# avi2924/Speech-Intent-Recognizer

Hardware: AMD Instinct MI355X
Metric: utterances/sec (16 kHz, 3 s clips), inference: HIP STFT+mel+CNN/BiGRU forward + argmax (higher is better)
Workload: dtype f32

## Files before the change

speech-intent-recognizer_amd/csrc/conv_fwd.h:

```cpp
#pragma once
#include "conv_wino2_f16x3_kernel.h"

template <int CIN, int COUT, int OUT_MODE>
static inline int conv_fwd(sir_handle* h, hipStream_t st, bool wino, const Wino2Geo& geo, int nb, const float* x, const unsigned short* w_wino,
                           const unsigned short* w_fallback, const float* scale, const float* shift, float* out, float2* stats,
                           const int* ctab = nullptr, int ncol_max = 0) {
    static_assert((CIN == 32 && COUT == 64) || (CIN == 64 && COUT == 128), "conv2 or conv3");
    const int H = geo.H, W = geo.W;
    if (wino) {
        SIR_TRY(sir_lds_opt_in(h, (const void*)conv3x3_wino2_f16x3_kernel<CIN, COUT, OUT_MODE, 0, 3>, W2_LDS_BYTES));
        SIR_HIP_TRY((launch_conv_wino2<CIN, COUT, OUT_MODE>(st, geo, x, w_wino, scale, shift, out, stats, h->zero_page, h->num_cus, ctab, ncol_max)));
    } else if constexpr (CIN == 32) {
        hipLaunchKernelGGL((conv3x3_wino_bf16x6_kernel<CIN, COUT, OUT_MODE == 2 ? 2 : 0>), dim3(((W + 1) / 2 + 1) / 2, 1, nb), dim3(256), WINO_LDS_BYTES, st,
                           x, w_wino, scale, shift, out, H, W, H / 2, W / 2, OUT_MODE == 2 ? stats : (float2*)nullptr);
    } else {
        hipLaunchKernelGGL((conv3x3_bf16x6_ns_kernel<CIN, COUT, 2, 2, OUT_MODE, 0, 2, 1, 1>), dim3((W + 7) / 8, 1, nb), dim3(256), conv_ns_lds_bytes(2, 2, 2), st,
                           x, w_fallback, scale, shift, out, H, W, H / 2, W / 2, stats);
    }
    return SIR_OK;
}
```

speech-intent-recognizer_amd/csrc/conv_wino2_f16x3_kernel.h:

```cpp
#pragma once
#include "conv_wino_bf16x6_kernel.h"
#include "wino2_geo.h"

constexpr int W2_RS = 11;
constexpr int W2_NPOS = 18 * W2_RS;
constexpr int W2_RAW_PIECES = (W2_NPOS * 4 + 63) / 64;
constexpr int W2_RAW_BYTES = W2_RAW_PIECES * 1024;
constexpr int W2_PLB = 16 * 1024;
constexpr int W2_NRAW = 3;
constexpr int W2_V_BYTES = 2 * W2_PLB;
constexpr int W2_XCH_BYTES = 3 * W2_PLB;
constexpr int W2_LDS_BYTES = 2 * W2_V_BYTES + W2_NRAW * W2_RAW_BYTES + W2_XCH_BYTES;
constexpr int W2_THREADS = 768;
constexpr int W2_PPW = (W2_RAW_PIECES + 3) / 4;

__device__ __forceinline__ int w2_div(int n, const W2Div& d) {
    const unsigned un = (unsigned)n;
    if (d.pow2) return (int)(un >> d.sh);
    const unsigned t = __umulhi(d.m, un);
    return (int)((t + ((un - t) >> 1)) >> d.sh);
}

__device__ __forceinline__ void split_w_f16x3(float u, unsigned short& p0, unsigned short& p1, unsigned int* status) {
    constexpr float LIM = 31.984375f;
    if (status && !(fabsf(u) <= LIM)) __hip_atomic_fetch_or(status, 8u, __ATOMIC_RELAXED, __HIP_MEMORY_SCOPE_AGENT);
    u = __builtin_fminf(__builtin_fmaxf(u, -LIM), LIM);
    const _Float16 hi = (_Float16)u;
    const _Float16 lo = (_Float16)((u - (float)hi) * H3_LO_SCALE);
    p0 = __builtin_bit_cast(unsigned short, hi);
    p1 = __builtin_bit_cast(unsigned short, lo);
}
__device__ __forceinline__ void prep_conv_w_wino_f16x3_elem(const float* __restrict__ w, unsigned short* __restrict__ wpb, int cin, int cout, int idx,
                                                            unsigned int* status) {
    const int total = cin * 16 * cout;
    if (idx >= total) return;
    const int e = idx & 15, co = (idx >> 4) % cout, g = (idx >> 4) / cout;
    const int ci = (g / 16) * 16 + e, f = g % 16, i = f >> 2, j = f & 3;
    const float* gk = w + ((size_t)co * cin + ci) * 9;
    const float Gm[4][3] = {{1.f, 0.f, 0.f}, {.5f, .5f, .5f}, {.5f, -.5f, .5f}, {0.f, 0.f, 1.f}};
    float u = 0.0f;
#pragma unroll
    for (int k = 0; k < 3; ++k) {
        float t = 0.0f;
#pragma unroll
        for (int l = 0; l < 3; ++l) t = fmaf(gk[k * 3 + l], Gm[j][l], t);
        u = fmaf(Gm[i][k], t, u);
    }
    if (j == 3) u = -u;
    split_w_f16x3(u, wpb[idx], wpb[(size_t)total + idx], status);
}
static __global__ void prep_conv_w_wino_f16x3_kernel(const float* __restrict__ w, unsigned short* __restrict__ wpb, int cin, int cout,
                                                     unsigned int* status) {
    prep_conv_w_wino_f16x3_elem(w, wpb, cin, cout, blockIdx.x * blockDim.x + threadIdx.x, status);
}
__device__ __forceinline__ void prep_conv_wT_wino_f16x3_elem(const float* __restrict__ w, unsigned short* __restrict__ wpb, int cin_f, int cout_f,
                                                             int idx, unsigned int* status) {
    const int total = cout_f * 16 * cin_f;
    if (idx >= total) return;
    const int e = idx & 15, cop = (idx >> 4) % cin_f, g = (idx >> 4) / cin_f;
    const int co_f = (g / 16) * 16 + e, f = g % 16, i = f >> 2, j = f & 3;
    const float* gk = w + ((size_t)co_f * cin_f + cop) * 9;
    const float Gm[4][3] = {{1.f, 0.f, 0.f}, {.5f, .5f, .5f}, {.5f, -.5f, .5f}, {0.f, 0.f, 1.f}};
    float u = 0.0f;
#pragma unroll
    for (int k = 0; k < 3; ++k) {
        float t = 0.0f;
#pragma unroll
        for (int l = 0; l < 3; ++l) t = fmaf(gk[8 - (k * 3 + l)], Gm[j][l], t);
        u = fmaf(Gm[i][k], t, u);
    }
    if (j == 3) u = -u;
    split_w_f16x3(u, wpb[idx], wpb[(size_t)total + idx], status);
}
static __global__ void prep_conv_wT_wino_f16x3_kernel(const float* __restrict__ w, unsigned short* __restrict__ wpb, int cin_f, int cout_f,
                                                       unsigned int* status) {
    prep_conv_wT_wino_f16x3_elem(w, wpb, cin_f, cout_f, blockIdx.x * blockDim.x + threadIdx.x, status);
}

typedef float w2_f32x4 __attribute__((ext_vector_type(4)));
typedef unsigned w2_u32x2 __attribute__((ext_vector_type(2)));
__device__ __forceinline__ void w2_barrier() { asm volatile("s_waitcnt lgkmcnt(0)\n\ts_barrier" ::: "memory"); }
__device__ __forceinline__ void w2_read_row(unsigned base, w2_f32x4& r0, w2_f32x4& r1, w2_f32x4& r2, w2_f32x4& r3) {
    asm volatile("ds_read_b128 %0, %4\n\tds_read_b128 %1, %4 offset:64\n\tds_read_b128 %2, %4 offset:128\n\tds_read_b128 %3, %4 offset:192"
                 : "=&v"(r0), "=&v"(r1), "=&v"(r2), "=&v"(r3) : "v"(base) : "memory");
}
template <int OFF>
__device__ __forceinline__ void w2_write64(unsigned base, uint2 v) {
    const w2_u32x2 d = {v.x, v.y};
    asm volatile("ds_write_b64 %0, %1 offset:%2" :: "v"(base), "v"(d), "n"(OFF) : "memory");
}

__device__ long long w2_dbg_stamps[2][32];
__device__ long long w2_dbg_fine[8][8];
template <int CIN, int COUT, int OUT_MODE, int DBG = 0, int PRIO = 3>
__global__ __launch_bounds__(W2_THREADS, 3) void conv3x3_wino2_f16x3_kernel(
    const float* __restrict__ x, const unsigned short* __restrict__ wpb, const float* __restrict__ scale,
    const float* __restrict__ shift, float* __restrict__ out, Wino2Geo geo, float2* __restrict__ stats, const float* __restrict__ zeros) {
    constexpr int NCH = CIN / 16, G = NCH * 16, NCHO = COUT >= 64 ? COUT / 64 : 1;
    static_assert(CIN % 16 == 0 && (COUT % 64 == 0 || COUT == 32), "16-channel chunks; 64-channel tasks (32: the n = 1 consumer waves only keep the barriers)");
    static_assert(NCH >= 2, "a task's exchange pieces are read behind its closing barrier; the next task's are written >= one barrier later");
    extern __shared__ __attribute__((aligned(1024))) unsigned char w2s[];
    constexpr int VB = W2_V_BYTES;
    unsigned char* const vbuf = w2s;
    unsigned char* const rawbuf = w2s + 2 * VB;
    unsigned char* const xchbuf = rawbuf + W2_NRAW * W2_RAW_BYTES;

    const int tid = threadIdx.x, lane = tid & 63, wv = __builtin_amdgcn_readfirstlane(tid >> 6);
    const bool producer = wv < 4;
    const int H = geo.H, W = geo.W, TW = geo.TW, NG = geo.NG, RBN = geo.RBN;
    const int* const ctab = OUT_MODE <= 1 ? geo.ctab : nullptr;
    const int NS = ctab ? RBN * ctab[0] : geo.NS;
    const int ntask_s = (NS - (int)blockIdx.x + (int)gridDim.x - 1) / (int)gridDim.x;
    const int ntask = ntask_s * NCHO;
    if (ntask <= 0) return;
    const int nsteps = ntask * NCH;

    auto task_geo = [&](int lt, int& g0, int& ty0, int& ch, int& s) {
        s = (int)blockIdx.x + (lt / NCHO) * (int)gridDim.x;
        ch = lt % NCHO;
        const int cb = w2_div(s, geo.dRBN), rb = s - cb * RBN;
        g0 = ctab ? ctab[1 + cb] : 4 * cb; ty0 = 8 * rb;
    };
    constexpr bool IDLE_DMA = COUT < 64;
    constexpr int D_STRIDE = 4, D_PPW = (W2_RAW_PIECES + D_STRIDE - 1) / D_STRIDE;
    const int d_stride = D_STRIDE;
    const int d_rank = producer ? wv : ((wv - 4) >> 1);
    int pre_lr[D_PPW], pre_lc[D_PPW], pre_part[D_PPW];
#pragma unroll
    for (int ii = 0; ii < D_PPW; ++ii) {
        const int slot = 64 * (d_rank + d_stride * ii) + lane, pos = slot >> 2, sp = slot & 3;
        const int lr = pos / W2_RS;
        const int lc = pos - lr * W2_RS - ((lr >> 1) & 1);
        const bool hole = lr > 17 || lc < 0 || lc > 9;
        pre_lr[ii] = hole ? (1 << 20) : lr;
        pre_lc[ii] = lc;
        pre_part[ii] = (sp ^ (((lr >> 2) & 1) << 1)) * 4;
    }
    auto raw_offsets = [&](int g0, int ty0, unsigned (&off)[D_PPW]) {
        const int plo = ctab ? 2 * TW * w2_div(g0, geo.dTW) : 0, phi = ctab ? plo + W : 2 * NG;
#pragma unroll
        for (int ii = 0; ii < D_PPW; ++ii) {
            const int gy = 2 * ty0 - 1 + pre_lr[ii];
            const int P = 2 * g0 - 1 + pre_lc[ii];
            const int Pc = min(max(P, 0), 2 * NG - 1);
            const int bb = w2_div(Pc, geo.d2TW), px = Pc - bb * 2 * TW;
            const bool ok = gy >= 0 && gy < H && P >= plo && P < phi && px < W;
            off[ii] = ok ? (unsigned)(((bb * H + gy) * W + px) * CIN + pre_part[ii]) : ~0u;
        }
    };
        auto raw_issue = [&](const unsigned (&off)[D_PPW], int c, int slot_buf) {
#pragma unroll
        for (int ii = 0; ii < D_PPW; ++ii) {
            const int k = d_rank + d_stride * ii;
            if (k < W2_RAW_PIECES) {
                const float* src = off[ii] == ~0u ? zeros : x + off[ii];
                __builtin_amdgcn_global_load_lds((sir_gptr_t)(src + c * 16), (sir_lptr_t)(rawbuf + slot_buf * W2_RAW_BYTES + k * 1024), 16, 0, 0);
            }
        }
    };
    int ig0, ity0, ich, is_;
    unsigned roff[D_PPW];
    int roff_task = -1;
    auto issue_chunk = [&](int q) {
        if (q >= nsteps) return;
        const int lt = q / NCH, c = q - lt * NCH;
        if (lt != roff_task) { task_geo(lt, ig0, ity0, ich, is_); raw_offsets(ig0, ity0, roff); roff_task = lt; }
        raw_issue(roff, c, q % W2_NRAW);
    };
    int nst = 0;
    auto stamp = [&]() {
        if (DBG && blockIdx.x == 0 && lane == 0 && (wv == 0 || wv == 4) && nst < 32) w2_dbg_stamps[producer ? 0 : 1][nst] = __builtin_amdgcn_s_memtime();
        ++nst;
    };

    if (producer) {
        if (PRIO) __builtin_amdgcn_s_setprio(PRIO);
        __builtin_amdgcn_s_setreg((1 ) | (23 << 6) | (0 << 11), 1);
        const int wg = wv;
        const int tR = wg >> 1, tH = wg & 1, tm = lane >> 1, tP1 = lane & 1;
        const int tty = tm & 7, ttx = tm >> 3, tpart = 2 * tH + tP1;
        unsigned ra_rel[3];
#pragma unroll
        for (int rr = 0; rr < 3; ++rr) {
            const int lr = 2 * tty + tR + rr;
            ra_rel[rr] = (unsigned)((lr * W2_RS + 2 * ttx + ((lr >> 1) & 1)) * 64 + ((tpart ^ (((lr >> 2) & 1) << 1)) * 16));
        }
        const unsigned raw_a = (unsigned)(uintptr_t)rawbuf, v_a = (unsigned)(uintptr_t)vbuf + (8 * tR) * 1024 + tH * 512 + tm * 16 + tP1 * 8;
        if (!IDLE_DMA) {
            issue_chunk(0);
            issue_chunk(1);
            asm volatile("s_waitcnt vmcnt(0)" ::: "memory");
        }
        w2_barrier();
        bool edge = false, z0 = false, z3 = false;
        auto fine = [&](int s_, int k_) {
            if (DBG && blockIdx.x == 0 && lane == 0 && wv == 0 && s_ >= 8 && s_ < 16) w2_dbg_fine[s_ - 8][k_] = __builtin_amdgcn_s_memtime();
        };
#pragma unroll 1
        for (int s = 0; s <= nsteps; ++s) {
            stamp();
            fine(s, 0);
            if (s < nsteps) {
                if (!IDLE_DMA && !(DBG & 2)) issue_chunk(s + 2);
                fine(s, 1);
                if (s % NCH == 0) {
                    int cg0, cty0, cch, cs;
                    task_geo(s / NCH, cg0, cty0, cch, cs);
                    const int t0 = cg0 - w2_div(cg0, geo.dTW) * TW;
                    edge = !ctab && (t0 == 0 || t0 + 3 >= TW - 1);
                    const int txx = (t0 + ttx) - w2_div(t0 + ttx, geo.dTW) * TW;
                    z0 = txx == 0; z3 = txx == TW - 1;
                }
                const unsigned rb = raw_a + (s % W2_NRAW) * W2_RAW_BYTES, vd = v_a + (s & 1) * VB;
                if (!(DBG & 4)) {
                w2_f32x4 q[3][4];
#pragma unroll
                for (int rr = 0; rr < 3; ++rr) w2_read_row(rb + ra_rel[rr], q[rr][0], q[rr][1], q[rr][2], q[rr][3]);
                asm volatile("s_waitcnt lgkmcnt(0)" ::: "memory");
                fine(s, 2);
                if (edge) {
                    asm volatile("" ::: "memory");
                    const w2_f32x4 zero4 = {0.0f, 0.0f, 0.0f, 0.0f};
#pragma unroll
                    for (int rr = 0; rr < 3; ++rr) { q[rr][0] = z0 ? zero4 : q[rr][0]; q[rr][3] = z3 ? zero4 : q[rr][3]; }
                }
                auto rows = [&](auto trc) {
                    constexpr int TR = decltype(trc)::value;
#pragma unroll
                    for (int il = 0; il < 2; ++il) {
                        w2_f32x4 R[4];
#pragma unroll
                        for (int j = 0; j < 4; ++j) {
                            if (TR == 0) R[j] = il == 0 ? q[0][j] - q[2][j] : q[1][j] + q[2][j];
                            else         R[j] = il == 0 ? q[1][j] - q[0][j] : q[0][j] - q[2][j];
                        }
                        const w2_f32x4 V[4] = {R[0] - R[2], R[1] + R[2], R[2] - R[1], R[1] - R[3]};
#pragma unroll
                        for (int j = 0; j < 4; ++j) {
                            const unsigned d = vd + (4 * il + j) * 1024;
                            uint2 sh, sl;
                            split2h_pair_ovfl(V[j].x, V[j].y, sh.x, sl.x);
                            split2h_pair_ovfl(V[j].z, V[j].w, sh.y, sl.y);
                            w2_write64<0>(d, sh);
                            w2_write64<W2_PLB>(d, sl);
                        }
                    }
                };
                if (tR == 0) rows(std::integral_constant<int, 0>{});
                else rows(std::integral_constant<int, 1>{});
                if (DBG) asm volatile("s_waitcnt lgkmcnt(0)" ::: "memory");
                fine(s, 3);
                }
                if (!IDLE_DMA) {
                    if (s + 2 < nsteps) asm volatile("s_waitcnt vmcnt(%0)" :: "n"(W2_RAW_PIECES / 4) : "memory");
                    else asm volatile("s_waitcnt vmcnt(0)" ::: "memory");
                }
            }
            stamp();
            fine(s, 4);
            w2_barrier();
            fine(s, 5);
        }
        return;
    }

    const int cw = wv - 4, mn = cw & 1, mi = cw >> 1, m = lane & 31, h = lane >> 5;
    if (COUT < 64 && mn == 1) {
        if (IDLE_DMA) {
            if (!(DBG & 2)) { issue_chunk(0); issue_chunk(1); }
            asm volatile("s_waitcnt vmcnt(0)" ::: "memory");
            w2_barrier();
#pragma unroll 1
            for (int s = 0; s <= nsteps; ++s) {
                if (s < nsteps) {
                    if (!(DBG & 2)) issue_chunk(s + 2);
                    if (s + 2 < nsteps) asm volatile("s_waitcnt vmcnt(%0)" :: "n"(W2_RAW_PIECES / 4) : "memory");
                    else asm volatile("s_waitcnt vmcnt(0)" ::: "memory");
                }
                w2_barrier();
            }
            return;
        }
        w2_barrier();
        w2_barrier();
        for (int lt = 0; lt < ntask; ++lt)
            for (int c = 0; c < NCH; ++c) w2_barrier();
        return;
    }
    const unsigned wlane = (unsigned)((m * 2 + h) * 16);
    const unsigned char* const wbase = reinterpret_cast<const unsigned char*>(wpb) + (size_t)mn * 1024;
    constexpr int NPW = 2;
    uint4 wq[4][NPW];
    auto load_w = [&](int gidx, int chh, uint4 (&q)[NPW]) {
#pragma unroll
        for (int p = 0; p < NPW; ++p)
            q[p] = *reinterpret_cast<const uint4*>(wbase + ((size_t)(p * G + gidx) * (COUT * 2) + (size_t)chh * 128) * 16 + wlane);
    };
    int g0, ty0, ch, s_idx;
    task_geo(0, g0, ty0, ch, s_idx);
#pragma unroll
    for (int j = 0; j < 4; ++j) load_w(4 * mi + j, ch, wq[j]);
    f32x16 acc[4];
#pragma unroll
    for (int j = 0; j < 4; ++j)
#pragma unroll
        for (int r = 0; r < 16; ++r) acc[j][r] = 0.0f;
    w2_barrier();
    float run_s[NCHO], run_q[NCHO];
#pragma unroll
    for (int k = 0; k < NCHO; ++k) { run_s[k] = 0.0f; run_q[k] = 0.0f; }

    stamp();
    stamp();
    w2_barrier();
#pragma unroll 1
    for (int lt = 0; lt < ntask; ++lt) {
        int g0n = g0, ty0n = ty0, chn = ch, sn = s_idx;
        if (lt + 1 < ntask) task_geo(lt + 1, g0n, ty0n, chn, sn);
#pragma unroll 1
        for (int c = 0; c < NCH; ++c) {
            stamp();
            const int sc = lt * NCH + c;
            const bool task_end = c == NCH - 1;
            const unsigned char* abase = vbuf + (sc & 1) * VB + h * 512 + m * 16 + (4 * mi) * 1024;
            const int gnxt = (task_end ? 0 : c + 1) * 16 + 4 * mi;
#pragma unroll
            for (int jp = 0; jp < 2; ++jp) {
                constexpr int NPA = 2;
                bf16x8 a[2][NPA], bq[2][3];
#pragma unroll
                for (int jj = 0; jj < 2; ++jj) {
#pragma unroll
                    for (int p = 0; p < NPA; ++p)
                        a[jj][p] = __builtin_bit_cast(bf16x8, *reinterpret_cast<const uint4*>(abase + p * W2_PLB + (2 * jp + jj) * 1024));
                    const f16x8 uh = __builtin_bit_cast(f16x8, wq[2 * jp + jj][0]);
                    bq[jj][0] = __builtin_bit_cast(bf16x8, uh);
                    bq[jj][1] = __builtin_bit_cast(bf16x8, uh * (_Float16)2048.0f);
                    bq[jj][2] = __builtin_bit_cast(bf16x8, wq[2 * jp + jj][1]);
                }
                if (DBG & 8) {
#pragma unroll
                    for (int jj = 0; jj < 2; ++jj)
                        acc[2 * jp + jj][0] += __builtin_bit_cast(float4, a[jj][0]).x + __builtin_bit_cast(float4, a[jj][1]).y + __builtin_bit_cast(float4, a[jj][NPA - 1]).z +
                                               __builtin_bit_cast(float4, bq[jj][0]).x + __builtin_bit_cast(float4, bq[jj][1]).y + __builtin_bit_cast(float4, bq[jj][2]).z;
                } else {
                    constexpr int HA[3] = {1, 0, 0}, HB[3] = {0, 2, 1};
#pragma unroll
                    for (int t3 = 0; t3 < 3; ++t3)
#pragma unroll
                        for (int jj = 0; jj < 2; ++jj)
                            acc[2 * jp + jj] = __builtin_amdgcn_mfma_f32_32x32x16_f16(__builtin_bit_cast(f16x8, a[jj][HA[t3]]),
                                                                                      __builtin_bit_cast(f16x8, bq[jj][HB[t3]]), acc[2 * jp + jj], 0, 0, 0);
                }
#pragma unroll
                for (int jj = 0; jj < 2; ++jj) if (!(DBG & 64)) load_w(gnxt + 2 * jp + jj, task_end ? chn : ch, wq[2 * jp + jj]);
                __builtin_amdgcn_sched_barrier(0);
            }
            stamp();
            if (!task_end) w2_barrier();
        }
        if (DBG & 16) { w2_barrier(); if (acc[0][0] == 1234.5f && acc[1][1] + acc[2][2] + acc[3][3] == 4.0f) out[0] = 1.0f; }
        else {
            {
                float4* const xch = reinterpret_cast<float4*>(xchbuf);
                float own[2][4];
#pragma unroll
                for (int b = 0; b < 2; ++b) {
                    const f32x16 Wc = b == 0 ? acc[0] + acc[1] + acc[2] : acc[1] - acc[2] + acc[3];
#pragma unroll
                    for (int k = 0; k < 4; ++k) {
                        if (k == mi) {
#pragma unroll
                            for (int e = 0; e < 4; ++e) own[b][e] = Wc[4 * k + e];
                        } else {
                            float4* dst = xch + (size_t)((mn * 4 + mi) * 3 + ((k - mi - 1) & 3)) * 128 + lane;
                            dst[b * 64] = make_float4(Wc[4 * k], Wc[4 * k + 1], Wc[4 * k + 2], Wc[4 * k + 3]);
                        }
                    }
                }
                w2_barrier();
                float Y[2][2][4];
#pragma unroll
                for (int i = 0; i < 4; ++i) {
                    const int kk = (mi - i - 1) & 3;
                    const float4* src = xch + (size_t)((mn * 4 + i) * 3 + (kk < 3 ? kk : 0)) * 128 + lane;
#pragma unroll
                    for (int b = 0; b < 2; ++b) {
                        const float4 v = src[b * 64];
                        const float w[4] = {i == mi ? own[b][0] : v.x, i == mi ? own[b][1] : v.y, i == mi ? own[b][2] : v.z, i == mi ? own[b][3] : v.w};
#pragma unroll
                        for (int e = 0; e < 4; ++e) {
                            if (i == 0) Y[0][b][e] = w[e];
                            else if (i <= 2) Y[0][b][e] += w[e];
                            if (i == 1) Y[1][b][e] = w[e];
                            else if (i >= 2) Y[1][b][e] -= w[e];
                        }
                    }
                }
                const int co = ch * 64 + mn * 32 + m;
                float ssum = 0.0f, ssq = 0.0f;
                float sc_ = 1.0f, sh_ = 0.0f;
                constexpr float DESC = H3_LO_INV;
                if (OUT_MODE <= 1) { sc_ = scale[co] * DESC; sh_ = shift[co]; }
                {
                    const int gc = g0 + mi;
                    const int img = w2_div(gc, geo.dTW), tx = gc - img * TW;
                    const bool tvalid = gc < (ctab ? (w2_div(g0, geo.dTW) + 1) * TW : NG);
                    if (OUT_MODE <= 1) {
                        float pooled[4];
#pragma unroll
                        for (int e = 0; e < 4; ++e) {
                            float v = 0.0f;
#pragma unroll
                            for (int a = 0; a < 2; ++a)
#pragma unroll
                                for (int b = 0; b < 2; ++b) v = fmaxf(v, fmaf(Y[a][b][e], sc_, sh_));
                            pooled[e] = v;
                        }
                        if (tvalid && tx < geo.Wp) {
                            if (OUT_MODE == 0) {
#pragma unroll
                                for (int e = 0; e < 4; ++e)
                                    out[(((size_t)img * geo.Hp + ty0 + 4 * h + e) * geo.Wp + tx) * COUT + co] = pooled[e];
                            } else {
                                const size_t oidx = ((size_t)img * geo.Wp + tx) * (COUT * geo.Hp) + (size_t)co * geo.Hp + ty0 + 4 * h;
                                const float4 v4 = make_float4(pooled[0], pooled[1], pooled[2], pooled[3]);
                                *reinterpret_cast<float4*>(out + oidx) = v4;
                                if (stats) {
                                    unsigned short* planes = reinterpret_cast<unsigned short*>(stats);
                                    const size_t plane = (size_t)geo.B * geo.Wp * (COUT * geo.Hp);
                                    uint2 hh, ll;
                                    split2h_quad(v4, hh, ll);
                                    *reinterpret_cast<uint2*>(planes + oidx) = hh;
                                    *reinterpret_cast<uint2*>(planes + plane + oidx) = ll;
                                }
                            }
                        }
                    } else {
#pragma unroll
                        for (int e = 0; e < 4; ++e)
#pragma unroll
                            for (int a = 0; a < 2; ++a)
#pragma unroll
                                for (int b = 0; b < 2; ++b) {
                                    const int gy = 2 * (ty0 + 4 * h + e) + a, gx = 2 * tx + b;
                                    if (tvalid && gx < W) {
                                        const float v = Y[a][b][e] * DESC;
                                        out[(((size_t)img * H + gy) * W + gx) * COUT + co] = v;
                                        ssum += v;
                                        ssq = fmaf(v, v, ssq);
                                    }
                                }
                    }
                }
                if (OUT_MODE == 2) {
#pragma unroll
                    for (int k = 0; k < NCHO; ++k)
                        if (k == ch) { run_s[k] += ssum; run_q[k] += ssq; }
                }
            }
        }
        g0 = g0n; ty0 = ty0n; ch = chn; s_idx = sn;
#pragma unroll
        for (int j = 0; j < 4; ++j)
#pragma unroll
            for (int r = 0; r < 16; ++r) acc[j][r] = 0.0f;
    }
    if (OUT_MODE == 2 && stats) {
#pragma unroll
        for (int k = 0; k < NCHO; ++k) {
            float a = run_s[k], q = run_q[k];
            a += __shfl_xor(a, 32);
            q += __shfl_xor(q, 32);
            if (h == 0) stats[((size_t)blockIdx.x * 4 + mi) * COUT + k * 64 + mn * 32 + m] = make_float2(a, q);
        }
    }
}

template <int CIN, int COUT, int OUT_MODE, int DBG = 0, int PRIO = 3>
static inline hipError_t launch_conv_wino2(hipStream_t st, Wino2Geo g, const float* x, const unsigned short* wpb, const float* scale,
                                           const float* shift, float* out, float2* stats, const float* zeros, int max_wg = 256,
                                           const int* ctab = nullptr, int ncol_max = 0) {
    if (ctab) {
        if (OUT_MODE > 1 || ncol_max < 1) return hipErrorInvalidValue;
        g.ctab = ctab;
        g.NS = g.RBN * ncol_max;
    }
    const int nwg = g.NS < max_wg ? g.NS : max_wg;
    hipLaunchKernelGGL((conv3x3_wino2_f16x3_kernel<CIN, COUT, OUT_MODE, DBG, PRIO>), dim3(nwg), dim3(W2_THREADS), W2_LDS_BYTES, st, x, wpb, scale, shift, out, g, stats, zeros);
    return hipGetLastError();
}
```

speech-intent-recognizer_amd/csrc/model_infer.hip:

```cpp
#include "f16x3_kernels.h"
#include "conv_fwd.h"
#include "gru_frag_prep.h"

namespace {

enum WsBuf {
    WS_A1 = 0,
    WS_A2,
    WS_X0,
    WS_GI,
    WS_Y0,
    WS_Y1,
    WS_CTX,
    WS_PAD,
    WS_XZ,
    WS_BN,
    WS_WHT,
    WS_XS,
    WS_WS,
    WS_WCB,
    WS_GXB,
    WS_GFL,
    WS_COUNT
};

struct Dims : SirDims {
    int tw2, tw3, k2max, k3max;
};

bool make_dims(int batch, int t_frames, Dims* d) {
    if (!sir_make_dims(batch, t_frames, d)) return false;
    d->tw2 = (d->wp1 + 1) / 2; d->tw3 = (d->wp2 + 1) / 2; d->k2max = (d->tw2 + 3) / 4; d->k3max = (d->tw3 + 3) / 4;
    return true;
}

struct PadTabs { size_t e0, d1, d3, tab2, tab3, rows, count; };
PadTabs pad_tabs(const Dims& d) {
    PadTabs t;
    const size_t n = (size_t)d.B + 1;
    t.e0 = 0; t.d1 = d.B; t.d3 = t.d1 + n; t.tab2 = t.d3 + n; t.tab3 = t.tab2 + 1 + n * d.k2max; t.rows = t.tab3 + 1 + n * d.k3max;
    t.count = t.rows + 1 + n * d.S;
    return t;
}

void ws_sizes(const Dims& d, size_t* bytes) {
    const size_t B = d.B + 1;
    bytes[WS_A1] = B * 32 * d.wp1 * 32 * 4;
    bytes[WS_A2] = B * 16 * d.wp2 * 64 * 4;
    bytes[WS_X0] = B * d.S * 1024 * 4;
    bytes[WS_GI] = B * d.S * 1536 * 4;
    bytes[WS_Y0] = (size_t)d.B * d.S * 512 * 4;
    bytes[WS_Y1] = (size_t)d.B * d.S * 512 * 4;
    bytes[WS_CTX] = (size_t)d.B * 512 * 4;
    bytes[WS_PAD] = pad_tabs(d).count * 4;
    bytes[WS_XZ] = (size_t)64 * d.T * 4;
    bytes[WS_BN] = (size_t)2 * 224 * 4;
    bytes[WS_WHT] = 4 * GRU_FRAG_BYTES;
    bytes[WS_XS] = B * d.S * 1024 * 2 * 2;
    bytes[WS_WS] = ((size_t)2 * 2 * 768 * 1024 + (size_t)2 * 2 * 768 * 512) * 2;
    bytes[WS_WCB] = ((size_t)3 * 32 * 16 * 64 + (size_t)3 * 64 * 16 * 128 + (size_t)3 * 64 * 9 * 128) * 2;
    bytes[WS_GXB] = 0;
    bytes[WS_GFL] = 0;
}

size_t ws_layout(const Dims& d, size_t* off) {
    size_t bytes[WS_COUNT], pos = 0;
    ws_sizes(d, bytes);
    for (int i = 0; i < WS_COUNT; ++i) {
        off[i] = pos;
        pos += sir_align_up(bytes[i], 256);
    }
    return pos;
}

static __global__ __launch_bounds__(256) void pad_extent_kernel(const float* __restrict__ x, int T, int* __restrict__ e0) {
    const unsigned* xb = reinterpret_cast<const unsigned*>(x) + (size_t)blockIdx.x * 64 * T;
    int last = -1;
    for (int c = threadIdx.x; c < T; c += 256) {
        unsigned acc = 0;
#pragma unroll 32
        for (int r = 0; r < 64; ++r) acc |= xb[(size_t)r * T + c];
        if (acc) last = c;
    }
#pragma unroll
    for (int o = 32; o > 0; o >>= 1) last = max(last, __shfl_xor(last, o));
    __shared__ int wl[4];
    if ((threadIdx.x & 63) == 0) wl[threadIdx.x >> 6] = last;
    __syncthreads();
    if (threadIdx.x == 0) e0[blockIdx.x] = max(max(wl[0], wl[1]), max(wl[2], wl[3])) + 1;
}

static __global__ __launch_bounds__(1024) void pad_tables_kernel(const int* __restrict__ e0, Dims d, int* __restrict__ d1o, int* __restrict__ d3o,
                                                                 int* __restrict__ tab2, int* __restrict__ tab3, int* __restrict__ prow,
                                                                 float* __restrict__ xz) {
    const int tid = threadIdx.x;
    for (int i = tid; i < 64 * d.T; i += 1024) xz[i] = 0.0f;
    const int nu = d.B + 1, per = (nu + 1023) / 1024, u0 = min(nu, tid * per), u1 = min(nu, u0 + per);
    auto need = [&](int u, int& c1, int& c3, int& k2, int& k3) {
        if (u == d.B) { c1 = d.wp1; c3 = d.S; k2 = d.k2max; k3 = d.k3max; return; }
        c3 = min(d.S, (e0[u] + 14) / 8);
        const int c2 = min(d.wp2, 2 * c3 + 1);
        c1 = min(d.wp1, 2 * c2 + 1);
        k2 = (c2 + 3) / 4; k3 = (c3 + 3) / 4;
    };
    int s2 = 0, s3 = 0, sr = 0, c1, c3, k2, k3;
    for (int u = u0; u < u1; ++u) { need(u, c1, c3, k2, k3); s2 += k2; s3 += k3; sr += c3; }
    __shared__ int p2[1024], p3[1024], pr[1024];
    p2[tid] = s2; p3[tid] = s3; pr[tid] = sr;
    __syncthreads();
    for (int o = 1; o < 1024; o <<= 1) {
        const int a2 = tid >= o ? p2[tid - o] : 0, a3 = tid >= o ? p3[tid - o] : 0, ar = tid >= o ? pr[tid - o] : 0;
        __syncthreads();
        p2[tid] += a2; p3[tid] += a3; pr[tid] += ar;
        __syncthreads();
    }
    int o2 = p2[tid] - s2, o3 = p3[tid] - s3, orw = pr[tid] - sr;
    for (int u = u0; u < u1; ++u) {
        need(u, c1, c3, k2, k3);
        d1o[u] = c1; d3o[u] = c3;
        for (int k = 0; k < k2; ++k) tab2[1 + o2 + k] = u * d.tw2 + 4 * k;
        for (int k = 0; k < k3; ++k) tab3[1 + o3 + k] = u * d.tw3 + 4 * k;
        for (int s = 0; s < c3; ++s) prow[1 + orw + s] = u * d.S + s;
        o2 += k2; o3 += k3; orw += c3;
    }
    if (tid == 1023) { tab2[0] = p2[1023]; tab3[0] = p3[1023]; prow[0] = pr[1023]; }
}

}

extern "C" size_t sir_model_workspace_bytes(const sir_handle* h, int batch, int t_frames, int train) {
    (void)h;
    if (train) return sir_train_workspace_bytes_impl(batch, t_frames);
    Dims d;
    if (!make_dims(batch, t_frames, &d)) return 0;
    size_t off[WS_COUNT];
    return ws_layout(d, off);
}

extern "C" int sir_model_workspace_offsets(const sir_handle* h, int batch, int t_frames, int train, size_t* offsets,
                                           int n) {
    (void)h; (void)train;
    Dims d;
    if (!make_dims(batch, t_frames, &d) || !offsets) { sir_set_error("sir_model_workspace_offsets: bad shape"); return SIR_EINVAL; }
    size_t off[WS_COUNT];
    ws_layout(d, off);
    for (int i = 0; i < n && i < WS_COUNT; ++i) offsets[i] = off[i];
    return WS_COUNT;
}

extern "C" int sir_model_infer(sir_handle* h, const sir_model_weights* w, const float* feats, int batch, int t_frames,
                               float* logits, int64_t* argmax, void* workspace, size_t workspace_bytes, void* stream_) {
    if (!h || !w || !feats || !logits || !workspace) { sir_set_error("sir_model_infer: NULL argument"); return SIR_EINVAL; }
    Dims d;
    if (!make_dims(batch, t_frames, &d)) {
        sir_set_error("sir_model_infer: unsupported shape batch=%d t_frames=%d (need t_frames >= 8)", batch, t_frames);
        return SIR_EINVAL;
    }
    if (h->cfg.n_mels != 64) { sir_set_error("sir_model_infer: the model is wired for 64 mels (models.py:23)"); return SIR_EUNSUPPORTED; }
    if (w->num_classes < 1 || w->num_classes > 64) { sir_set_error("sir_model_infer: num_classes=%d", w->num_classes); return SIR_EINVAL; }
    size_t off[WS_COUNT];
    const size_t need = ws_layout(d, off);
    if (workspace_bytes < need) { sir_set_error("sir_model_infer: workspace %zu < %zu", workspace_bytes, need); return SIR_ENOMEM; }
    if (((uintptr_t)workspace & 255) != 0) { sir_set_error("sir_model_infer: workspace must be 256-byte aligned"); return SIR_EINVAL; }
    hipStream_t st = (hipStream_t)stream_;
    char* ws = (char*)workspace;
    float* a1 = (float*)(ws + off[WS_A1]);
    float* a2 = (float*)(ws + off[WS_A2]);
    float* x0 = (float*)(ws + off[WS_X0]);
    float* gi = (float*)(ws + off[WS_GI]);
    float* y0 = (float*)(ws + off[WS_Y0]);
    float* y1 = (float*)(ws + off[WS_Y1]);
    float* ctx = (float*)(ws + off[WS_CTX]);
    float* bns = (float*)(ws + off[WS_BN]);
    float* bnt = bns + 224;
    float* wht = (float*)(ws + off[WS_WHT]);
    unsigned short* xs = (unsigned short*)(ws + off[WS_XS]);
    unsigned short* wsl0 = (unsigned short*)(ws + off[WS_WS]);
    unsigned short* wsl1 = wsl0 + (size_t)2 * 2 * 768 * 1024;
    unsigned short* wcb2 = (unsigned short*)(ws + off[WS_WCB]);
    unsigned short* wcb3 = wcb2 + (size_t)3 * 32 * 16 * 64;
    unsigned short* wcb3d = wcb3 + (size_t)3 * 64 * 16 * 128;
    const int B = d.B, S = d.S;
    const PadTabs pt = pad_tabs(d);
    int* const ptab = (int*)(ws + off[WS_PAD]);
    float* const xz = (float*)(ws + off[WS_XZ]);

    const SirConvPlan cp = sir_conv_plan(&d, true);
    const bool w2 = cp.fwd_wino;
    const int BT = w2 ? B + 1 : B;

    const long long prep_key = ((long long)B << 32) | (unsigned)d.T;
    sir_handle::PrepEntry* pe = nullptr;
    for (auto& e : h->prep)
        if (e.ws == workspace) pe = &e;
    const bool reuse_prep = pe && h->weights_version != 0 && pe->version == h->weights_version && pe->key == prep_key;
    if (!reuse_prep) {
        SirProfScope prof(h, SIR_K_PREP, st);
        const int bn_c[3] = {32, 64, 128}, bn_o[3] = {0, 32, 96};
        for (int i = 0; i < 3; ++i)
            hipLaunchKernelGGL(prep_bn_kernel, dim3(1), dim3(128), 0, st, w->bn_w[i], w->bn_b[i], w->bn_mean[i], w->bn_var[i],
                               bns + bn_o[i], bnt + bn_o[i], bn_c[i]);
        for (int i = 0; i < 4; ++i) sir_prep_whh_quad(st, w->gru_w_hh[i], (unsigned char*)wht + (size_t)i * GRU_FRAG_BYTES);
        if (w2) hipLaunchKernelGGL(prep_conv_w_wino_f16x3_kernel, dim3((32 * 16 * 64 + 255) / 256), dim3(256), 0, st, w->conv_w[1], wcb2, 32, 64, h->status);
        else hipLaunchKernelGGL(prep_conv_w_wino_bf16x3_kernel, dim3((32 * 16 * 64 + 255) / 256), dim3(256), 0, st, w->conv_w[1], wcb2, 32, 64);
        if (w2) hipLaunchKernelGGL(prep_conv_w_wino_f16x3_kernel, dim3((64 * 16 * 128 + 255) / 256), dim3(256), 0, st, w->conv_w[2], wcb3, 64, 128, h->status);
        else hipLaunchKernelGGL(prep_conv_w_wino_bf16x3_kernel, dim3((64 * 16 * 128 + 255) / 256), dim3(256), 0, st, w->conv_w[2], wcb3, 64, 128);
        hipLaunchKernelGGL(prep_conv_w_bf16x3_kernel, dim3((64 * 9 * 128 + 255) / 256), dim3(256), 0, st, w->conv_w[2], wcb3d, 64, 128);
        for (int dir = 0; dir < 2; ++dir) {
            hipLaunchKernelGGL(split2h_kernel, dim3(384), dim3(256), 0, st, w->gru_w_ih[dir], 1024, wsl0 + (size_t)dir * 2 * 768 * 1024, (size_t)768, 1024);
            hipLaunchKernelGGL(split2h_kernel, dim3(192), dim3(256), 0, st, w->gru_w_ih[2 + dir], 512, wsl1 + (size_t)dir * 2 * 768 * 512, (size_t)768, 512);
        }
        if (!pe) { pe = &h->prep[h->prep_next]; h->prep_next = (h->prep_next + 1) % 4; }
        pe->ws = workspace; pe->version = h->weights_version; pe->key = prep_key;
    }
    SIR_KCHECK();

    {
        SirProfScope prof(h, SIR_K_CONV1, st);
        if (w2) {
            hipLaunchKernelGGL(pad_extent_kernel, dim3(B), dim3(256), 0, st, feats, d.T, ptab + pt.e0);
            hipLaunchKernelGGL(pad_tables_kernel, dim3(1), dim3(1024), 0, st, (const int*)(ptab + pt.e0), d, ptab + pt.d1, ptab + pt.d3,
                               ptab + pt.tab2, ptab + pt.tab3, ptab + pt.rows, xz);
        }
        hipLaunchKernelGGL(conv1_mfma_bn_relu_pool_kernel, dim3((d.wp1 + C1_PCOLS - 1) / C1_PCOLS, 1, BT), dim3(256), 0, st, feats,
                           w->conv_w[0], bns, bnt, a1, 64, d.T, 32, d.wp1, (const float*)xz, B, w2 ? (const int*)(ptab + pt.d1) : (const int*)nullptr);
    }
    {
        SirProfScope prof(h, SIR_K_CONV2, st);
        SIR_TRY((conv_fwd<32, 64, 0>(h, st, w2, cp.geo2, BT, a1, wcb2, nullptr, bns + 32, bnt + 32, a2, nullptr, ptab + pt.tab2, (B + 1) * d.k2max)));
    }
    {
        SirProfScope prof(h, SIR_K_CONV3, st);
        SIR_TRY((conv_fwd<64, 128, 1>(h, st, w2, cp.geo3, BT, a2, wcb3, wcb3d, bns + 96, bnt + 96, x0, (float2*)xs, ptab + pt.tab3, (B + 1) * d.k3max)));
    }
    SIR_KCHECK();

    const int M = B * S;
    {
        SirProfScope prof(h, SIR_K_GEMM_IH0, st);
        if (w2)
            SIR_TRY(launch_gemm_nt_f16x3_gather(h, st, (const unsigned short*)xs, (const unsigned short*)wsl0,
                                                    (const unsigned short*)(wsl0 + (size_t)2 * 768 * 1024), w->gru_b_ih[0], w->gru_b_ih[1], gi, 1536,
                                                    (const int*)(ptab + pt.rows), BT * S, 768, 1024));
        else
            SIR_TRY(launch_gemm_nt_f16x3(h, st, (const unsigned short*)xs, (const unsigned short*)wsl0,
                                             (const unsigned short*)(wsl0 + (size_t)2 * 768 * 1024), w->gru_b_ih[0], w->gru_b_ih[1], gi, 1536, M, 768, 1024));
    }
    {
        SirProfScope prof(h, SIR_K_GRU0, st);
        SIR_TRY(sir_launch_gru_quad(h, st, false, gi, w->gru_w_hh[0], w->gru_w_hh[1], w->gru_b_hh[0], w->gru_b_hh[1], y0, B, S, nullptr,
                                    xs, wht, (unsigned char*)wht + GRU_FRAG_BYTES, w2 ? (const int*)(ptab + pt.d3) : (const int*)nullptr));
    }
    {
        SirProfScope prof(h, SIR_K_GEMM_IH1, st);
        SIR_TRY(launch_gemm_nt_f16x3(h, st, (const unsigned short*)xs, (const unsigned short*)wsl1,
                                         (const unsigned short*)(wsl1 + (size_t)2 * 768 * 512), w->gru_b_ih[2], w->gru_b_ih[3], gi, 1536, M, 768, 512));
    }
    {
        SirProfScope prof(h, SIR_K_GRU1, st);
        SIR_TRY(sir_launch_gru_quad(h, st, false, gi, w->gru_w_hh[2], w->gru_w_hh[3], w->gru_b_hh[2], w->gru_b_hh[3], y1, B, S, nullptr,
                                    nullptr, (unsigned char*)wht + 2 * GRU_FRAG_BYTES, (unsigned char*)wht + 3 * GRU_FRAG_BYTES));
    }
    SIR_KCHECK();

    {
        SirProfScope prof(h, SIR_K_ATTN, st);
        hipLaunchKernelGGL(attention_pool_kernel, dim3(B), dim3(256), 0, st, y1, w->attn_w, w->attn_b, ctx, S, w->fc_w, w->fc_b,
                           w->num_classes, logits, (long long*)argmax);
    }
    SIR_KCHECK();
    return SIR_OK;
}
```

speech-intent-recognizer_amd/csrc/wino2_geo.h:

```cpp
#pragma once
#include <stddef.h>

struct W2Div { unsigned m; int sh; int pow2; unsigned d; };
static inline W2Div w2_div_make(unsigned d) {
    W2Div r{0u, 0, 0, d};
    if ((d & (d - 1)) == 0) { r.pow2 = 1; while ((1u << r.sh) < d) ++r.sh; return r; }
    int l = 0;
    while ((1ull << l) < d) ++l;
    r.m = (unsigned)((((1ull << l) - d) << 32) / d + 1);
    r.sh = l - 1;
    return r;
}

struct Wino2Geo {
    int H, W;
    int TW;
    int NG;
    int RBN;
    int NS;
    int Hp, Wp;
    int B;
    W2Div dTW, d2TW, dRBN;
    const int* ctab;
};
static inline bool wino2_geo(int B, int H, int W, int cmax, Wino2Geo* g) {
    g->B = B; g->H = H; g->W = W; g->TW = (W + 1) / 2; g->NG = B * g->TW; g->RBN = H / 16; g->ctab = nullptr;
    g->NS = g->RBN * ((g->NG + 3) / 4); g->Hp = H / 2; g->Wp = W / 2;
    g->dTW = w2_div_make((unsigned)g->TW); g->d2TW = w2_div_make(2u * (unsigned)g->TW); g->dRBN = w2_div_make((unsigned)(g->RBN > 0 ? g->RBN : 1));
    return H % 16 == 0 && W >= 1 && B >= 1 && (size_t)B * H * W * cmax < ((size_t)1 << 31) && (size_t)g->NG * 2 < ((size_t)1 << 30);
}
static inline size_t wino2_stat_blocks(int B, int H, int W, int max_wg) {
    const size_t ns = (size_t)(H / 16) * (((size_t)B * ((W + 1) / 2) + 3) / 4);
    return (ns < (size_t)max_wg ? ns : (size_t)max_wg) * 4;
}
```

Baseline: 739,000.

## Dynamically claim Winograd conv tasks via a global atomic counter

Replaces the static strided task assignment in the persistent Winograd conv kernel with dynamic work stealing. After two statically assigned tasks, each workgroup claims further tasks through a global atomic counter. One lane issues the claim two chunks ahead and publishes it to a small LDS ring, so the fetch overlaps with the DMA pipeline. The counters are zeroed in the pad-tables kernel. This targets load imbalance from the padded/compacted column tables, at the cost of atomic traffic, an extra vmcnt slot and LDS reads per task. It also adds a trace-analysis script.

```diff
diff --git a/devtools/trace_pipeline.py b/devtools/trace_pipeline.py
--- /dev/null
+++ b/devtools/trace_pipeline.py
@@ -0,0 +1,128 @@
+import csv
+import statistics
+import sys
+from collections import defaultdict
+
+SEGMENT_GAP_NS = 2_000_000
+
+
+def short(name):
+    n = name.replace("(anonymous namespace)::", "")
+    if n.startswith("void "):
+        n = n[5:]
+    n = n.split("(")[0]
+    return n[:64]
+
+
+def load(path):
+    rows = list(csv.DictReader(open(path)))
+    key = "Stream_Id" if rows and "Stream_Id" in rows[0] and len({r["Stream_Id"] for r in rows}) > 1 else "Queue_Id"
+    ev = [(int(r["Start_Timestamp"]), int(r["End_Timestamp"]), short(r["Kernel_Name"]), r[key]) for r in rows]
+    ev.sort()
+    return ev, key
+
+
+def overlaps(ev):
+    out = []
+    by_start = ev
+    for i, (s, e, n, q) in enumerate(by_start):
+        ov = gru = False
+        j = i - 1
+        while j >= 0 and by_start[j][0] > s - 5_000_000:
+            s2, e2, n2, q2 = by_start[j]
+            if q2 != q and e2 > s:
+                ov = True
+                gru = gru or n2.startswith("gru_quad_kernel")
+            j -= 1
+        j = i + 1
+        while not ov and j < len(by_start) and by_start[j][0] < e:
+            ov = by_start[j][3] != q
+            j += 1
+        out.append((ov, gru))
+    return out
+
+
+def sweep(ev, t0, t1):
+    pts = []
+    for s, e, n, _ in ev:
+        if e <= t0 or s >= t1:
+            continue
+        g = n.startswith("gru_quad_kernel")
+        pts.append((max(s, t0), 1, g))
+        pts.append((min(e, t1), -1, g))
+    pts.sort(key=lambda p: (p[0], p[1]))
+    idle = only = 0
+    act = gact = 0
+    prev = t0
+    for t, d, g in pts:
+        if act == 0:
+            idle += t - prev
+        elif act == gact:
+            only += t - prev
+        act += d
+        gact += d if g else 0
+        prev = t
+    idle += t1 - prev
+    return idle, only
+
+
+def main(path):
+    ev, key = load(path)
+    ovl = overlaps(ev)
+    open_b = defaultdict(list)
+    batches = []
+    for i, (s, e, n, q) in enumerate(ev):
+        open_b[q].append(i)
+        if n.startswith("attention_pool_kernel"):
+            idx = open_b.pop(q)
+            batches.append((ev[idx[0]][0], e, q, idx))
+    batches.sort(key=lambda b: b[1])
+    piped = [b for b in batches if any(ovl[i][0] for i in b[3])]
+    if not piped:
+        sys.exit("no batch overlaps a kernel of another stream: not a pipelined trace")
+    segs, cur = [], [piped[0]]
+    for b in piped[1:]:
+        if b[1] - cur[-1][1] > SEGMENT_GAP_NS:
+            segs.append(cur)
+            cur = []
+        cur.append(b)
+    segs.append(cur)
+    segs = [s for s in segs if len(s) >= 4]
+    nb = sum(len(s) - 1 for s in segs)
+    wall = sum(s[-1][1] - s[0][1] for s in segs)
+    idle = only = 0
+    for s in segs:
+        a, b = sweep(ev, s[0][1], s[-1][1])
+        idle += a
+        only += b
+    print(f"streams keyed by {key}; {len(batches)} batches, {len(piped)} pipelined in {len(segs)} segments")
+    print(f"pipelined, per batch: wall {wall / nb / 1e3:.1f} us, nothing running {idle / nb / 1e3:.1f} us, "
+          f"only gru_quad_kernel running {only / nb / 1e3:.1f} us")
+    per = defaultdict(lambda: [0, 0])
+    conv = defaultdict(lambda: {"ovl": [], "alone": [], "beside_gru": 0, "n": 0})
+    seg_batches = {id(b) for s in segs for b in s[1:]}
+    for b in batches:
+        for i in b[3]:
+            s, e, n, q = ev[i]
+            if id(b) in seg_batches:
+                per[n][0] += e - s
+                per[n][1] += 1
+            if n.startswith("conv3x3_wino2_f16x3_kernel"):
+                c = conv[n]
+                (c["ovl"] if ovl[i][0] else c["alone"]).append(e - s)
+                if id(b) in seg_batches:
+                    c["n"] += 1
+                    c["beside_gru"] += ovl[i][1]
+    print("summed kernel time per pipelined batch:")
+    for n, (t, c) in sorted(per.items(), key=lambda kv: -kv[1][0]):
+        print(f"  {n:64s} {c / nb:5.2f} x {t / c / 1e3:7.1f} us = {t / nb / 1e3:7.1f} us")
+    print(f"  {'sum':64s} {'':17s} {sum(t for t, _ in per.values()) / nb / 1e3:7.1f} us")
+    for n, c in sorted(conv.items()):
+        med = lambda v: statistics.median(v) / 1e3 if v else float("nan")
+        print(f"{n}: overlapped median {med(c['ovl']):.1f} us (n = {len(c['ovl'])}, min {min(c['ovl'] or [0]) / 1e3:.1f}, "
+              f"max {max(c['ovl'] or [0]) / 1e3:.1f}), alone median {med(c['alone']):.1f} us (n = {len(c['alone'])}); "
+              f"{c['beside_gru']} of {c['n']} pipelined launches begin beside a gru_quad_kernel of another stream")
+
+
+if __name__ == "__main__":
+    main(sys.argv[1])
diff --git a/speech-intent-recognizer_amd/csrc/conv_fwd.h b/speech-intent-recognizer_amd/csrc/conv_fwd.h
--- a/speech-intent-recognizer_amd/csrc/conv_fwd.h
+++ b/speech-intent-recognizer_amd/csrc/conv_fwd.h
@@ -4,12 +4,12 @@
 template <int CIN, int COUT, int OUT_MODE>
 static inline int conv_fwd(sir_handle* h, hipStream_t st, bool wino, const Wino2Geo& geo, int nb, const float* x, const unsigned short* w_wino,
                            const unsigned short* w_fallback, const float* scale, const float* shift, float* out, float2* stats,
-                           const int* ctab = nullptr, int ncol_max = 0) {
+                           const int* ctab = nullptr, int ncol_max = 0, int* ctr = nullptr) {
     static_assert((CIN == 32 && COUT == 64) || (CIN == 64 && COUT == 128), "conv2 or conv3");
     const int H = geo.H, W = geo.W;
     if (wino) {
         SIR_TRY(sir_lds_opt_in(h, (const void*)conv3x3_wino2_f16x3_kernel<CIN, COUT, OUT_MODE, 0, 3>, W2_LDS_BYTES));
-        SIR_HIP_TRY((launch_conv_wino2<CIN, COUT, OUT_MODE>(st, geo, x, w_wino, scale, shift, out, stats, h->zero_page, h->num_cus, ctab, ncol_max)));
+        SIR_HIP_TRY((launch_conv_wino2<CIN, COUT, OUT_MODE>(st, geo, x, w_wino, scale, shift, out, stats, h->zero_page, h->num_cus, ctab, ncol_max, ctr)));
     } else if constexpr (CIN == 32) {
         hipLaunchKernelGGL((conv3x3_wino_bf16x6_kernel<CIN, COUT, OUT_MODE == 2 ? 2 : 0>), dim3(((W + 1) / 2 + 1) / 2, 1, nb), dim3(256), WINO_LDS_BYTES, st,
                            x, w_wino, scale, shift, out, H, W, H / 2, W / 2, OUT_MODE == 2 ? stats : (float2*)nullptr);
diff --git a/speech-intent-recognizer_amd/csrc/conv_wino2_f16x3_kernel.h b/speech-intent-recognizer_amd/csrc/conv_wino2_f16x3_kernel.h
--- a/speech-intent-recognizer_amd/csrc/conv_wino2_f16x3_kernel.h
+++ b/speech-intent-recognizer_amd/csrc/conv_wino2_f16x3_kernel.h
@@ -10,7 +10,8 @@
 constexpr int W2_NRAW = 3;
 constexpr int W2_V_BYTES = 2 * W2_PLB;
 constexpr int W2_XCH_BYTES = 3 * W2_PLB;
-constexpr int W2_LDS_BYTES = 2 * W2_V_BYTES + W2_NRAW * W2_RAW_BYTES + W2_XCH_BYTES;
+constexpr int W2_TQ_SLOTS = 8;
+constexpr int W2_LDS_BYTES = 2 * W2_V_BYTES + W2_NRAW * W2_RAW_BYTES + W2_XCH_BYTES + W2_TQ_SLOTS * 4;
 constexpr int W2_THREADS = 768;
 constexpr int W2_PPW = (W2_RAW_PIECES + 3) / 4;
 
@@ -88,6 +89,20 @@
 __device__ __forceinline__ void w2_write64(unsigned base, uint2 v) {
     const w2_u32x2 d = {v.x, v.y};
     asm volatile("ds_write_b64 %0, %1 offset:%2" :: "v"(base), "v"(d), "n"(OFF) : "memory");
+}
+
+__device__ __forceinline__ int w2_read_word(unsigned addr) {
+    int v;
+    asm volatile("ds_read_b32 %0, %1\n\ts_waitcnt lgkmcnt(0)" : "=v"(v) : "v"(addr) : "memory");
+    return __builtin_amdgcn_readfirstlane(v);
+}
+
+__device__ __forceinline__ void w2_claim_issue(int* ctr, int& claimed) {
+    const int zero = 0, one = 1;
+    asm volatile("global_atomic_add %0, %1, %2, %3 sc0" : "+v"(claimed) : "v"(zero), "v"(one), "s"(ctr) : "memory");
+}
+__device__ __forceinline__ void w2_claim_publish(unsigned lds_addr, int& claimed) {
+    asm volatile("ds_write_b32 %1, %0" : "+v"(claimed) : "v"(lds_addr) : "memory");
 }
 
 __device__ long long w2_dbg_stamps[2][32];
@@ -110,16 +125,31 @@
     const int H = geo.H, W = geo.W, TW = geo.TW, NG = geo.NG, RBN = geo.RBN;
     const int* const ctab = OUT_MODE <= 1 ? geo.ctab : nullptr;
     const int NS = ctab ? RBN * ctab[0] : geo.NS;
+    constexpr bool CLAIMF = OUT_MODE <= 1 && COUT >= 64;
+    constexpr int LA = 2;
+    static_assert(W2_RAW_PIECES / 4 == 3 && (W2_RAW_PIECES - 1) % 4 != 3, "the claiming wave (3) issues 3 pieces per chunk");
+    const bool dyn = CLAIMF && ctab && geo.ctr;
+    const int ntotal = NS * NCHO;
     const int ntask_s = (NS - (int)blockIdx.x + (int)gridDim.x - 1) / (int)gridDim.x;
-    const int ntask = ntask_s * NCHO;
+    int ntask = dyn ? ((int)blockIdx.x < ntotal ? 0x3fffffff / NCH : 0) : ntask_s * NCHO;
     if (ntask <= 0) return;
-    const int nsteps = ntask * NCH;
-
+    int nsteps = ntask * NCH;
+    const unsigned tq_a = (unsigned)(uintptr_t)(w2s + W2_LDS_BYTES - W2_TQ_SLOTS * 4);
+    const int claim_base = LA * (int)gridDim.x;
+
+    auto task_id = [&](int lt) { return lt < LA ? (int)blockIdx.x + lt * (int)gridDim.x : claim_base + w2_read_word(tq_a + (lt & (W2_TQ_SLOTS - 1)) * 4); };
     auto task_geo = [&](int lt, int& g0, int& ty0, int& ch, int& s) {
-        s = (int)blockIdx.x + (lt / NCHO) * (int)gridDim.x;
-        ch = lt % NCHO;
+        if (dyn) {
+            const int id = task_id(lt);
+            if ((unsigned)id >= (unsigned)ntotal) return false;
+            s = id / NCHO; ch = id % NCHO;
+        } else {
+            s = (int)blockIdx.x + (lt / NCHO) * (int)gridDim.x;
+            ch = lt % NCHO;
+        }
         const int cb = w2_div(s, geo.dRBN), rb = s - cb * RBN;
         g0 = ctab ? ctab[1 + cb] : 4 * cb; ty0 = 8 * rb;
+        return true;
     };
     constexpr bool IDLE_DMA = COUT < 64;
     constexpr int D_STRIDE = 4, D_PPW = (W2_RAW_PIECES + D_STRIDE - 1) / D_STRIDE;
@@ -164,7 +194,11 @@
     auto issue_chunk = [&](int q) {
         if (q >= nsteps) return;
         const int lt = q / NCH, c = q - lt * NCH;
-        if (lt != roff_task) { task_geo(lt, ig0, ity0, ich, is_); raw_offsets(ig0, ity0, roff); roff_task = lt; }
+        if (lt != roff_task) {
+            if (!task_geo(lt, ig0, ity0, ich, is_)) { nsteps = lt * NCH; return; }
+            raw_offsets(ig0, ity0, roff);
+            roff_task = lt;
+        }
         raw_issue(roff, c, q % W2_NRAW);
     };
     int nst = 0;
@@ -193,6 +227,9 @@
         }
         w2_barrier();
         bool edge = false, z0 = false, z3 = false;
+        const bool claimer = dyn && wv == 3 && lane == 0;
+        bool claim_flying = false;
+        int claimed = 0, claim_slot = 0;
         auto fine = [&](int s_, int k_) {
             if (DBG && blockIdx.x == 0 && lane == 0 && wv == 0 && s_ >= 8 && s_ < 16) w2_dbg_fine[s_ - 8][k_] = __builtin_amdgcn_s_memtime();
         };
@@ -202,12 +239,18 @@
             fine(s, 0);
             if (s < nsteps) {
                 if (!IDLE_DMA && !(DBG & 2)) issue_chunk(s + 2);
+                claim_flying = false;
+                if (CLAIMF && s % NCH == NCH - 2) {
+                    claim_flying = claimer && s + 2 < nsteps;
+                    if (claim_flying) w2_claim_issue(geo.ctr, claimed);
+                    claim_slot = (s / NCH + 2) & (W2_TQ_SLOTS - 1);
+                }
                 fine(s, 1);
-                if (s % NCH == 0) {
+                if (!ctab && s % NCH == 0) {
                     int cg0, cty0, cch, cs;
                     task_geo(s / NCH, cg0, cty0, cch, cs);
                     const int t0 = cg0 - w2_div(cg0, geo.dTW) * TW;
-                    edge = !ctab && (t0 == 0 || t0 + 3 >= TW - 1);
+                    edge = t0 == 0 || t0 + 3 >= TW - 1;
                     const int txx = (t0 + ttx) - w2_div(t0 + ttx, geo.dTW) * TW;
                     z0 = txx == 0; z3 = txx == TW - 1;
                 }
@@ -252,9 +295,11 @@
                 fine(s, 3);
                 }
                 if (!IDLE_DMA) {
-                    if (s + 2 < nsteps) asm volatile("s_waitcnt vmcnt(%0)" :: "n"(W2_RAW_PIECES / 4) : "memory");
-                    else asm volatile("s_waitcnt vmcnt(0)" ::: "memory");
-                }
+                    if (s + 2 >= nsteps) asm volatile("s_waitcnt vmcnt(0)" ::: "memory");
+                    else if (claim_flying) asm volatile("s_waitcnt vmcnt(%0)" :: "n"(W2_RAW_PIECES / 4 + 1) : "memory");
+                    else asm volatile("s_waitcnt vmcnt(%0)" :: "n"(W2_RAW_PIECES / 4) : "memory");
+                }
+                if (CLAIMF && s % NCH == NCH - 1 && claimer) w2_claim_publish(tq_a + claim_slot * 4, claimed);
             }
             stamp();
             fine(s, 4);
@@ -316,7 +361,9 @@
 #pragma unroll 1
     for (int lt = 0; lt < ntask; ++lt) {
         int g0n = g0, ty0n = ty0, chn = ch, sn = s_idx;
-        if (lt + 1 < ntask) task_geo(lt + 1, g0n, ty0n, chn, sn);
+        if (dyn) {
+            if (!task_geo(lt + 1, g0n, ty0n, chn, sn)) ntask = lt + 1;
+        } else if (lt + 1 < ntask) task_geo(lt + 1, g0n, ty0n, chn, sn);
 #pragma unroll 1
         for (int c = 0; c < NCH; ++c) {
             stamp();
@@ -480,10 +527,12 @@
 template <int CIN, int COUT, int OUT_MODE, int DBG = 0, int PRIO = 3>
 static inline hipError_t launch_conv_wino2(hipStream_t st, Wino2Geo g, const float* x, const unsigned short* wpb, const float* scale,
                                            const float* shift, float* out, float2* stats, const float* zeros, int max_wg = 256,
-                                           const int* ctab = nullptr, int ncol_max = 0) {
+                                           const int* ctab = nullptr, int ncol_max = 0, int* ctr = nullptr) {
+    if (ctr && !ctab) return hipErrorInvalidValue;
     if (ctab) {
         if (OUT_MODE > 1 || ncol_max < 1) return hipErrorInvalidValue;
         g.ctab = ctab;
+        g.ctr = ctr;
         g.NS = g.RBN * ncol_max;
     }
     const int nwg = g.NS < max_wg ? g.NS : max_wg;
diff --git a/speech-intent-recognizer_amd/csrc/model_infer.hip b/speech-intent-recognizer_amd/csrc/model_infer.hip
--- a/speech-intent-recognizer_amd/csrc/model_infer.hip
+++ b/speech-intent-recognizer_amd/csrc/model_infer.hip
@@ -34,12 +34,13 @@
     return true;
 }
 
-struct PadTabs { size_t e0, d1, d3, tab2, tab3, rows, count; };
+struct PadTabs { size_t e0, d1, d3, tab2, tab3, rows, ctr, count; };
 PadTabs pad_tabs(const Dims& d) {
     PadTabs t;
     const size_t n = (size_t)d.B + 1;
     t.e0 = 0; t.d1 = d.B; t.d3 = t.d1 + n; t.tab2 = t.d3 + n; t.tab3 = t.tab2 + 1 + n * d.k2max; t.rows = t.tab3 + 1 + n * d.k3max;
-    t.count = t.rows + 1 + n * d.S;
+    t.ctr = t.rows + 1 + n * d.S;
+    t.count = t.ctr + 2;
     return t;
 }
 
@@ -92,8 +93,9 @@
 
 static __global__ __launch_bounds__(1024) void pad_tables_kernel(const int* __restrict__ e0, Dims d, int* __restrict__ d1o, int* __restrict__ d3o,
                                                                  int* __restrict__ tab2, int* __restrict__ tab3, int* __restrict__ prow,
-                                                                 float* __restrict__ xz) {
+                                                                 float* __restrict__ xz, int* __restrict__ ctr) {
     const int tid = threadIdx.x;
+    if (tid < 2) ctr[tid] = 0;
     for (int i = tid; i < 64 * d.T; i += 1024) xz[i] = 0.0f;
     const int nu = d.B + 1, per = (nu + 1023) / 1024, u0 = min(nu, tid * per), u1 = min(nu, u0 + per);
     auto need = [&](int u, int& c1, int& c3, int& k2, int& k3) {
@@ -220,18 +222,18 @@
         if (w2) {
             hipLaunchKernelGGL(pad_extent_kernel, dim3(B), dim3(256), 0, st, feats, d.T, ptab + pt.e0);
             hipLaunchKernelGGL(pad_tables_kernel, dim3(1), dim3(1024), 0, st, (const int*)(ptab + pt.e0), d, ptab + pt.d1, ptab + pt.d3,
-                               ptab + pt.tab2, ptab + pt.tab3, ptab + pt.rows, xz);
+                               ptab + pt.tab2, ptab + pt.tab3, ptab + pt.rows, xz, ptab + pt.ctr);
         }
         hipLaunchKernelGGL(conv1_mfma_bn_relu_pool_kernel, dim3((d.wp1 + C1_PCOLS - 1) / C1_PCOLS, 1, BT), dim3(256), 0, st, feats,
                            w->conv_w[0], bns, bnt, a1, 64, d.T, 32, d.wp1, (const float*)xz, B, w2 ? (const int*)(ptab + pt.d1) : (const int*)nullptr);
     }
     {
         SirProfScope prof(h, SIR_K_CONV2, st);
-        SIR_TRY((conv_fwd<32, 64, 0>(h, st, w2, cp.geo2, BT, a1, wcb2, nullptr, bns + 32, bnt + 32, a2, nullptr, ptab + pt.tab2, (B + 1) * d.k2max)));
+        SIR_TRY((conv_fwd<32, 64, 0>(h, st, w2, cp.geo2, BT, a1, wcb2, nullptr, bns + 32, bnt + 32, a2, nullptr, ptab + pt.tab2, (B + 1) * d.k2max, ptab + pt.ctr)));
     }
     {
         SirProfScope prof(h, SIR_K_CONV3, st);
-        SIR_TRY((conv_fwd<64, 128, 1>(h, st, w2, cp.geo3, BT, a2, wcb3, wcb3d, bns + 96, bnt + 96, x0, (float2*)xs, ptab + pt.tab3, (B + 1) * d.k3max)));
+        SIR_TRY((conv_fwd<64, 128, 1>(h, st, w2, cp.geo3, BT, a2, wcb3, wcb3d, bns + 96, bnt + 96, x0, (float2*)xs, ptab + pt.tab3, (B + 1) * d.k3max, ptab + pt.ctr + 1)));
     }
     SIR_KCHECK();
 
diff --git a/speech-intent-recognizer_amd/csrc/wino2_geo.h b/speech-intent-recognizer_amd/csrc/wino2_geo.h
--- a/speech-intent-recognizer_amd/csrc/wino2_geo.h
+++ b/speech-intent-recognizer_amd/csrc/wino2_geo.h
@@ -22,9 +22,10 @@
     int B;
     W2Div dTW, d2TW, dRBN;
     const int* ctab;
+    int* ctr;
 };
 static inline bool wino2_geo(int B, int H, int W, int cmax, Wino2Geo* g) {
-    g->B = B; g->H = H; g->W = W; g->TW = (W + 1) / 2; g->NG = B * g->TW; g->RBN = H / 16; g->ctab = nullptr;
+    g->B = B; g->H = H; g->W = W; g->TW = (W + 1) / 2; g->NG = B * g->TW; g->RBN = H / 16; g->ctab = nullptr; g->ctr = nullptr;
     g->NS = g->RBN * ((g->NG + 3) / 4); g->Hp = H / 2; g->Wp = W / 2;
     g->dTW = w2_div_make((unsigned)g->TW); g->d2TW = w2_div_make(2u * (unsigned)g->TW); g->dRBN = w2_div_make((unsigned)(g->RBN > 0 ? g->RBN : 1));
     return H % 16 == 0 && W >= 1 && B >= 1 && (size_t)B * H * W * cmax < ((size_t)1 << 31) && (size_t)g->NG * 2 < ((size_t)1 << 30);
```

After: 737,100. No clear change (-0.3%).
